# insight-platform/Similari

Hardware: NVIDIA H100
Metric: pair_associations_per_sec (higher is better)
Workload: dtype f32

## Files before the change

### similari_b200/csrc/engine.cu

```cuda
#include <cuda_runtime.h>

#include <algorithm>
#include <chrono>
#include <cmath>
#include <cstdlib>
#include <cstdarg>
#include <cstdio>
#include <cstring>
#include <map>
#include <string>
#include <type_traits>
#include <unordered_map>
#include <utility>
#include <vector>

#include "../../include/similari_b200.h"
#include "sb_engine.cuh"

#include <atomic>

namespace sb {
static std::atomic<unsigned long long> g_launches{0};
void note_launch(int n) { g_launches.fetch_add((unsigned long long)n, std::memory_order_relaxed); }
unsigned long long launch_count() { return g_launches.load(std::memory_order_relaxed); }
// ... 276 lines not shown
    }
    if (copy_stream) cudaStreamDestroy(copy_stream);
    if (side_stream) cudaStreamDestroy(side_stream);
    if (prep_stream) cudaStreamDestroy(prep_stream);
    for (cudaEvent_t e : {ev_user_in, ev_user_out, ev_prep_done, ev_set_free[0], ev_set_free[1], ev_inputs, ev_join_req, ev_cost_done}) if (e) cudaEventDestroy(e);
    for (auto& e : ev_fork) if (e) cudaEventDestroy(e);
    if (ev_join) cudaEventDestroy(ev_join);
    if (own_stream && stream) cudaStreamDestroy(stream);
  }

  template <auto F> static void in_ts(sb200_tracker& t, void* p) { t.ts.*F = static_cast<std::remove_reference_t<decltype(t.ts.*F)>>(p); }
  template <auto F> static void in_wb(sb200_tracker& t, void* p) { t.wb.*F = static_cast<std::remove_reference_t<decltype(t.wb.*F)>>(p); }

  std::vector<Col> store_table() {
    using TS = sb::TrackStore;
    const size_t K = (size_t)P.max_obs, d8 = (size_t)P.d8, H = (size_t)hist_len;
    std::vector<Col> c = {{&b_id, in_ts<&TS::id>, 8}, {&b_epoch, in_ts<&TS::epoch>, 4}, {&b_length, in_ts<&TS::length>, 4},
                          {&b_custom, in_ts<&TS::custom>, 8}, {&b_vt, in_ts<&TS::vt>, 1}, {&b_pred, in_ts<&TS::pred>, 24},
                          {&b_obs, in_ts<&TS::obs>, 24}, {&b_radius, in_ts<&TS::radius>, 4},
                          {&b_kst, in_ts<&TS::kst>, 4 * (size_t)sb::kStateStride}};
    if (P.positional_kind == SB200_POS_IOU) c.push_back({&b_vert, in_ts<&TS::vert>, 64});
    if (H > 1) {
      c.push_back({&b_hpred, in_ts<&TS::hist_pred>, 24 * H, true});
      c.push_back({&b_hobs, in_ts<&TS::hist_obs>, 24 * H, true});
    }
    if (P.is_visual) {
      c.push_back({&b_obs_phys, in_ts<&TS::obs_phys>, K, false, kRowTrack, kBlobAll, kTagObsPhys});
      c.push_back({&b_obs_hasf, in_ts<&TS::obs_hasf>, K});
      c.push_back({&b_obs_q, in_ts<&TS::obs_q>, 4 * K});
      c.push_back({&b_obs_n, in_ts<&TS::obs_n>, 1, false, kRowTrack, kBlobAll, kTagObsN});
      c.push_back({&b_feat_cnt, in_ts<&TS::feat_cnt>, 1});
      c.push_back({&b_fblk, in_ts<&TS::fblk>, 4, false, kRowTrack, kBlobAll, kTagFblk});
      if (fhist_on) c.push_back({&b_hblk, in_ts<&TS::hblk>, 4, false, kRowTrack, kBlobTrackerOnly, kTagHblk});
      c.push_back({&b_feat, in_ts<&TS::feat>, 4 * K * d8, false, kRowBlock});
      c.push_back({&b_feat_bf16, in_ts<&TS::feat_bf16>, 2 * K * d8, false, kRowBlock});
      c.push_back({&b_fnorm2, in_ts<&TS::fnorm2>, 4 * K, false, kRowBlock});
      if (P.d8 <= sb::kFp8MaxD8) {
        c.push_back({&b_feat_fp8, in_ts<&TS::feat_fp8>, K * sb::fp8_pitch(P.d8), false, kRowBlock, kBlobNo});
        c.push_back({&b_fscale, in_ts<&TS::fscale>, 4 * K, false, kRowBlock, kBlobNo});
      }
      c.push_back({&b_blk_owner, in_ts<&TS::blk_owner>, 4, false, kRowBlock, kBlobAll, kTagOwner});
      c.push_back({&b_blk_free, in_ts<&TS::blk_free>, 4, false, kRowFree, kBlobAll, kTagFree});
    }
    return c;
  }

  std::vector<Col> slot_table() {
    using TS = sb::TrackStore;
    return {{&b_ntracks, nullptr, 4, true}, {&b_cur_epoch, nullptr, 4, true}, {&b_scene_ids, nullptr, 8, true},
            {&b_nfree, in_ts<&TS::n_free>, 4, true}, {&b_atop, in_ts<&TS::arena_top>, 4, true}};
  }

  std::vector<Col> wasted_table() {
    using WB = sb::WastedBuf;
    const size_t H = (size_t)hist_len;
    std::vector<Col> c = {{&w_id, in_wb<&WB::id>, 8, false, kRowWasted}, {&w_scene, in_wb<&WB::scene>, 8, false, kRowWasted},
                          {&w_epoch, in_wb<&WB::epoch>, 4, false, kRowWasted}, {&w_length, in_wb<&WB::length>, 4, false, kRowWasted},
                          {&w_pred, in_wb<&WB::pred>, 24, false, kRowWasted}, {&w_obs, in_wb<&WB::obs>, 24, false, kRowWasted}};
    if (H > 1) {
      c.push_back({&w_hpred, in_wb<&WB::hist_pred>, 24 * H, false, kRowWasted});
      c.push_back({&w_hobs, in_wb<&WB::hist_obs>, 24 * H, false, kRowWasted});
    }
    if (fhist_on) c.push_back({&w_hblk, in_wb<&WB::hblk>, 4, false, kRowWasted, kBlobAll, kTagHblk});
    return c;
  }

  std::vector<Col> pool_table() {
    using TS = sb::TrackStore;
// ... 6 lines not shown
  int regrow(DBuf& b, size_t w, size_t groups, size_t rows, size_t old_groups, size_t old_rows, bool zero) {
    const size_t bytes = std::max<size_t>(1, groups * rows * w);
    DBuf nb;
    int rc = nb.ensure(bytes);
    if (rc) return rc;
    if (zero) CU(cudaMemsetAsync(nb.p, 0, bytes, stream));
    if (b.p && old_groups > 0 && old_rows > 0) {
      if (old_groups == 1)
        CU(cudaMemcpyAsync(nb.p, b.p, old_rows * w, cudaMemcpyDeviceToDevice, stream));
      else
        CU(cudaMemcpy2DAsync(nb.p, rows * w, b.p, old_rows * w, old_rows * w, old_groups, cudaMemcpyDeviceToDevice, stream));
      CU(cudaStreamSynchronize(stream));
    }
    b = std::move(nb);
    return 0;
  }

  int grow(const std::vector<Col>& cols, size_t groups, size_t rows, size_t old_groups, size_t old_rows) {
    for (const Col& c : cols) {
      const int rc = regrow(*c.buf, c.w, groups, rows, old_groups, old_rows, c.zero);
      if (rc) return rc;
      if (c.point) c.point(*this, c.buf->p);
    }
    return 0;
  }

  int regen_fp8(int slot, int top) {
    if (!ts.feat_fp8 || top <= 0) return 0;
    const long long r0 = (long long)slot * track_cap * P.max_obs, rows = (long long)top * P.max_obs;
    sb::launch_to_fp8(ts.feat + r0 * P.d8, P.d8, P.d8, P.d8, rows, ts.feat_fp8 + r0 * sb::fp8_pitch(P.d8), ts.fscale + r0, stream);
    return cudaGetLastError() == cudaSuccess ? 0 : fail(SB200_ERR_CUDA, "e4m3 row conversion failed");
  }

  int ensure_store(int need_scenes, int need_tracks) {
    if (need_scenes <= scene_cap && need_tracks <= track_cap) return 0;
    int ns = scene_cap, nt = track_cap;
    if (need_scenes > ns) ns = std::max(need_scenes, std::max(4, ns * 2));
    if (need_tracks > nt) nt = std::max(need_tracks, std::max(64, nt * 2));
    int rc = grow(store_table(), ns, nt, scene_cap, track_cap);
    if (rc) return rc;
    if (ns != scene_cap && (rc = grow(slot_table(), ns, 1, scene_cap, 1))) return rc;
    ts.kst_stride = sb::kStateStride;
    if (hist_len > 1) ts.hist_len = hist_len;
    scene_cap = ns;
    track_cap = nt;
    ts.track_cap = nt;
    return 0;
  }

  int slot_for(uint64_t scene_id, bool create) {
    auto it = slot_of.find(scene_id);
    if (it != slot_of.end()) return it->second;
    if (!create) return -1;
    int s = (int)scene_of_slot.size();
    slot_of[scene_id] = s;
    scene_of_slot.push_back(scene_id);
    epoch.push_back(0);
    n_tracks.push_back(0);
    n_hidden.push_back(0);
    arena_top.push_back(0);
    pending_add.push_back(0);
    return s;
  }

  int ensure_wasted(int64_t need) {
    if (need <= wb.cap) return 0;
    int64_t ncap = std::max<int64_t>(need, std::max<int64_t>(1024, (int64_t)wb.cap * 3));
    int rc = grow(wasted_table(), 1, (size_t)ncap, 1, (size_t)wasted_count);
    if (rc) return rc;
    if (!w_count.p) {
      if ((rc = w_count.ensure(sizeof(int)))) return rc;
      CU(cudaMemsetAsync(w_count.p, 0, sizeof(int), stream));
// ... 440 lines not shown
    if (fhist_on && (rc = ENS(f_histdst, T * 4))) return rc;
    if ((rc = ENS(cb.flags, T)) || (rc = ENS(cb.norm2, T * 4)) || (rc = ENS(f_featdst, T * 4)) ||
        (rc = ENS(f_vis, std::max<size_t>(4, (size_t)vis_total * 4))) || (rc = ENS(f_scene_max, 4 * (size_t)n_scenes)))
      return rc;
  }
  sb::TcArgs tc;
  memset(&tc, 0, sizeof(tc));
  tc.num_sms = num_sms;
  int mstep = 0, cstep = 256;
  const long long visl_alloc = std::max(visl_total, hint_dets * 64);
  if (want_tc || want_dense) {
    tc.use_tc = true;
    tc.dense = want_dense;
    mstep = 256;
    cstep = want_dense ? (256 / K) * K : sb::vis_screen_ucols(P.d8, num_sms, n_scenes, m_of.data(), nb_ub.data(), K);
    tc.cstep = cstep;
    long long tiles_ub = 0, slabs_ub = 0, ws_ub = 0, blk_ub = 0;
    for (int s = 0; s < n_scenes; ++s) {
      const long long ct = ((long long)nb_ub[s] * K + cstep - 1) / cstep;
      tiles_ub += (long long)((m_of[s] + mstep - 1) / mstep) * ct;
      slabs_ub += ct;
      ws_ub += ct * (cstep / K) * ((m_of[s] + 127) / 128 * 128);
      blk_ub += ct * (cstep / K);
    }
    tc.n_tiles = (int)tiles_ub;
    long long tiles_alloc = tiles_ub;
    {
      const long long hs = std::max(opts.max_scenes_hint, n_scenes), hd = std::max(opts.max_dets_per_scene_hint, max_m);
      const long long ht = std::max(hint_tracks, max_nb);
      tiles_alloc = std::max(tiles_alloc, hs * ((hd + mstep - 1) / mstep) * ((ht * K + cstep - 1) / cstep + 1));
      if (f_tiles.bytes > 0 && sizeof(sb::TcTile) * (size_t)tiles_alloc > f_tiles.bytes) tiles_alloc += tiles_alloc / 2;
    }
    const bool alloc8 = !want_dense && P.d8 <= sb::kFp8MaxD8 && ts.feat_fp8 != nullptr;
    if (alloc8 && ((rc = ENS(cb.fp8, T * sb::fp8_pitch(P.d8))) || (rc = ENS(cb.scale, T * 4)))) return rc;
    if ((rc = ENS(cb.bf16, T * P.d8 * 2)) || (rc = ENS(f_tiles, sizeof(sb::TcTile) * (size_t)std::max<long long>(1, tiles_alloc))) ||
        (rc = ENS(f_rowmeta, sizeof(sb::VisRowMeta) * (T + 256))))
      return rc;
    tc.rowmeta = f_rowmeta.as<sb::VisRowMeta>();
    tc.max_rows = max_nb * K;
    tc.d_tiles = f_tiles.as<sb::TcTile>();
    tc.d_n_tiles = &f_dyn.as<sb::FrameDyn>()->n_tiles;
    tc.a_rows = total;
    tc.b_rows = (long long)scene_cap * track_cap * K;
    if (!want_dense) {
      if ((rc = ENS(f_colmeta, sizeof(sb::VisColMeta) * (size_t)(std::max(col_total, hint_cols) + 256))) ||
          (rc = ENS(f_colb, 4 * (size_t)(std::max(col_total, hint_cols) + 256))) ||
          (rc = ENS(f_colvalid, (size_t)(std::max(col_total, hint_cols) + 256) / 8 + 16)) ||
          (rc = ENS(f_colgeo, sizeof(sb::VisColGeo) * (size_t)std::max<long long>(1, P.n_constraints > 0 ? std::max(col_total, hint_cols) : 1))))
        return rc;
      tc.colmeta = f_colmeta.as<sb::VisColMeta>();
      tc.colgeo = f_colgeo.as<sb::VisColGeo>();
      tc.colb = f_colb.as<float>();
      tc.colvalid = f_colvalid.as<unsigned int>();
      tc.total_cols = (int)col_total;
      if (alloc8 && P.visual_kind != SB200_VIS_COSINE) {
        if ((rc = ENS(f_colsb, 4 * (size_t)(std::max(col_total, hint_cols) + 256)))) return rc;
        if (want_fp8) tc.colsb = f_colsb.as<float>();
      }
      tc.fp8 = want_fp8;
    } else {
      const long long hs = std::max(opts.max_scenes_hint, n_scenes), ht = hint_tracks;
      const long long hd = std::max(opts.max_dets_per_scene_hint, 0);
      ws_ub = std::max(ws_ub, hs * (ht + 256) * ((hd + 127) / 128 * 128));
      blk_ub = std::max(blk_ub, hs * (ht + 256));
      slabs_ub = std::max(slabs_ub, hs * ((ht * K + cstep - 1) / cstep + 1));
      if ((rc = ENS(f_drowb, 4 * 5 * T)) || (rc = ENS(f_dcolb, 4 * (size_t)std::max<long long>(1, blk_ub))) ||
          (rc = ENS(f_slabk, 4 * 256 * (size_t)std::max<long long>(1, slabs_ub))))
// ... 162 lines not shown
  } rollback{this, &q, true};

  const double ms_setup = since(t_begin);
  if (has_user_stream) {
    if (!ev_user_in) { CU(cudaEventCreateWithFlags(&ev_user_in, cudaEventDisableTiming)); CU(cudaEventCreateWithFlags(&ev_user_out, cudaEventDisableTiming)); }
    CU(cudaEventRecord(ev_user_in, user_stream));
    CU(cudaStreamWaitEvent(stream, ev_user_in, 0));
  }
  if (!device_io && !prefetched && total > 0) {
    const size_t n = (size_t)total;
    CU(cudaMemcpyAsync(sin->boxes.p, boxes, n * 24, cudaMemcpyHostToDevice, stream));
    if (f.in_feat) {
      CU(cudaMemcpyAsync(sin->feat.p, features, n * (size_t)P.feature_dim * feat_bytes(), cudaMemcpyHostToDevice, stream));
      if (f.in_hasf) CU(cudaMemcpyAsync(sin->hasf.p, has_feature, n, cudaMemcpyHostToDevice, stream));
    }
    if (f.in_quality) CU(cudaMemcpyAsync(sin->quality.p, quality, n * 4, cudaMemcpyHostToDevice, stream));
    if (f.in_custom) CU(cudaMemcpyAsync(sin->custom.p, custom_ids, n * 8, cudaMemcpyHostToDevice, stream));
    if (f.in_own) CU(cudaMemcpyAsync(sin->own.p, own_area, n * 4, cudaMemcpyHostToDevice, stream));
  }
  if (!side_stream) {
    int lo = 0, hi = 0;
    CU(cudaDeviceGetStreamPriorityRange(&lo, &hi));
    CU(cudaStreamCreateWithPriority(&side_stream, cudaStreamNonBlocking, hi));
    for (auto& e : ev_fork) CU(cudaEventCreateWithFlags(&e, cudaEventDisableTiming));
    CU(cudaEventCreateWithFlags(&ev_join, cudaEventDisableTiming));
  }
  if (!prep_stream) {
    int lo = 0, hi = 0;
    CU(cudaDeviceGetStreamPriorityRange(&lo, &hi));
    CU(cudaStreamCreateWithPriority(&prep_stream, cudaStreamNonBlocking, lo));
    CU(cudaEventCreateWithFlags(&ev_prep_done, cudaEventDisableTiming));
    CU(cudaEventCreateWithFlags(&ev_inputs, cudaEventDisableTiming));
  }
  const bool prep_ahead = !derive_own && total > 0;
  const bool side_setup = !derive_own && total > 0;
  cudaStream_t s_setup = stream;
  if (side_setup) {
    CU(cudaEventRecord(ev_fork[0], stream));
    CU(cudaStreamWaitEvent(side_stream, ev_fork[0], 0));
    s_setup = side_stream;
  }
  sb::launch_frame_setup(P, ts, f, reinterpret_cast<const sb::SceneReq*>(q.h_req.dp), n_scenes, b_ntracks.as<int>(), mstep,
                         cstep, tc.dense, f_tiles.as<sb::TcTile>(), f_dyn.as<sb::FrameDyn>(), f_counters.as<int>(), (int)n_counters, s_setup);
  tc.max_init_done = 1;
  if (side_setup && Pf.is_visual && tc.use_tc && !tc.dense && tc.n_tiles > 0 && max_m > 0 && max_n > 0 && f.in_feat) {
    sb::launch_vis_colmeta(Pf, ts, f, n_scenes, max_n, tc, side_stream);
    tc.colmeta_done = 1;
  }
  if (side_setup) CU(cudaEventRecord(ev_join, side_stream));
  CU(cudaEventRecord(q.ev[0], stream));
  if (derive_own) {
    sb::launch_own_area(f, n_scenes, max_m, f.in_boxes, f_own.as<float>(), f_ownovf.as<int>(),
                        reinterpret_cast<int2*>(f_ownovf.as<char>() + 16), stream);
    f.in_own = f_own.as<float>();
  }
  if (prep_ahead) {
    if (has_user_stream) CU(cudaStreamWaitEvent(prep_stream, ev_user_in, 0));
    if (!device_io) {
      if (prefetched) CU(cudaStreamWaitEvent(prep_stream, sin->ev, 0));
      else { CU(cudaEventRecord(ev_inputs, stream)); CU(cudaStreamWaitEvent(prep_stream, ev_inputs, 0)); }
    }
    if (set_busy[cset]) CU(cudaStreamWaitEvent(prep_stream, ev_set_free[cset], 0));
    if (cost_done_valid) CU(cudaStreamWaitEvent(prep_stream, ev_cost_done, 0));
    sb::launch_prep(Pf, f, n_scenes, max_m, prep_stream);
    CU(cudaEventRecord(ev_prep_done, prep_stream));
    CU(cudaStreamWaitEvent(stream, ev_prep_done, 0));
// ... 898 lines not shown
  int bad = 0;
  CU(cudaMemcpyAsync(&bad, d_bad, sizeof(int), cudaMemcpyDeviceToHost, t->stream));
  CU(cudaStreamSynchronize(t->stream));
  if (bad) return fail(SB200_ERR_INVALID, "the blob holds %d out-of-range block or observation indices", bad);
  return 0;
}

int set_slots(sb200_tracker* t, const std::vector<sb::XferSlot>& tab, int free0, int free_add, int top_add,
              unsigned long long id_min, bool raise_ids) {
  if (tab.empty()) return 0;
  DBuf d_tab;
  int rc = d_tab.ensure(tab.size() * sizeof(sb::XferSlot));
  if (rc) return rc;
  CU(cudaMemcpyAsync(d_tab.p, tab.data(), tab.size() * sizeof(sb::XferSlot), cudaMemcpyHostToDevice, t->stream));
  const int e = sb::launch_xfer_slots(d_tab.as<sb::XferSlot>(), (int)tab.size(), t->b_ntracks.as<int>(), t->ts.n_free,
                                      t->ts.arena_top, t->ts, free0, free_add, top_add,
                                      raise_ids ? t->b_idc.as<unsigned long long>() : nullptr, id_min, t->stream);
  if (e) return fail(SB200_ERR_CUDA, "slot update launch failed: %s", cudaGetErrorString((cudaError_t)e));
  CU(cudaStreamSynchronize(t->stream));
  return 0;
}

uint64_t read_id_counter(sb200_tracker* t, int* rc) {
  uint64_t v = 0;
  *rc = 0;
  if (!t->b_idc.p) return 0;
  cudaError_t e = cudaMemcpyAsync(&v, t->b_idc.p, 8, cudaMemcpyDeviceToHost, t->stream);
  if (e == cudaSuccess) e = cudaStreamSynchronize(t->stream);
  if (e != cudaSuccess) *rc = fail(SB200_ERR_CUDA, "id counter read failed: %s", cudaGetErrorString(e));
  return v;
}

int save_blob(sb200_tracker* t, uint32_t type, const std::vector<int>& slots, void* dst, size_t cap, size_t* bytes) {
  BlobHeader h;
  memset(&h, 0, sizeof(h));
  h.magic = kBlobMagic; h.version = kBlobVersion; h.type = type;
  h.opts = t->opts;
  h.feature_history = t->fhist_on; h.hist_len = t->hist_len; h.d8 = t->P.d8; h.n_scenes = (int32_t)slots.size();
  h.seen_features = t->seen_features;
  if (type == kBlobTracker) {
    h.adapt_dense = t->adapt_dense;
    h.auto_waste_counter = t->auto_waste_counter; h.auto_waste_periodicity = t->auto_waste_periodicity;
    h.scene_cap = t->scene_cap; h.track_cap = t->track_cap;
  }
  std::vector<BlobScene> table(slots.size());
  std::vector<SlotRows> rows(slots.size());
  for (size_t i = 0; i < slots.size(); ++i) {
    const int s = slots[i];
    const int blk = t->P.is_visual ? t->arena_top[s] : 0;
    table[i] = {t->scene_of_slot[s], t->epoch[s], t->n_tracks[s], type == kBlobTracker ? t->n_hidden[s] : 0, blk};
    rows[i] = {s, t->n_tracks[s], blk, t->P.is_visual ? blk - t->n_tracks[s] : 0};
    h.live_total += rows[i].n; h.blk_total += rows[i].blk; h.free_total += rows[i].fre;
  }
  if (type == kBlobTracker) {
    h.wasted_count = t->wasted_count; h.revealed = t->revealed;
    h.hpool_top = t->fhist_on ? t->hpool_top : 0; h.hpool_free = t->fhist_on ? t->hpool_free : 0;
    h.hpool_cap = t->fhist_on ? t->hpool_cap : 0;
  }
  int rc = 0;
  h.id_counter = read_id_counter(t, &rc);
  if (rc) return rc;
  const uint64_t total = lay_out(h, section_bytes(t, type, h.n_scenes, h.live_total, h.blk_total, h.free_total,
                                                  h.wasted_count, h.hpool_top, h.hpool_free));
  h.total_bytes = total;
  *bytes = (size_t)total;
  if (!dst || cap < total) return fail(SB200_ERR_CAPACITY, "the blob needs %llu bytes", (unsigned long long)total);
// ... 318 lines not shown
```

### similari_b200/csrc/kernels_state.cu

```cuda
#include <cuda_bf16.h>

#include <algorithm>
#include <type_traits>

#include "sb_engine.cuh"

namespace sb {

constexpr int AT = 512;

__device__ __forceinline__ void write_box(float* dst, const Box& b) {
  dst[0] = b.xc; dst[1] = b.yc; dst[2] = b.angle; dst[3] = b.aspect; dst[4] = b.height; dst[5] = b.conf;
}
__device__ __forceinline__ void write_box_row(float* dst, const Box& b) {
  float2* d2 = reinterpret_cast<float2*>(dst);
  d2[0] = make_float2(b.xc, b.yc); d2[1] = make_float2(b.angle, b.aspect); d2[2] = make_float2(b.height, b.conf);
}

__global__ void __launch_bounds__(AT) apply_rank_kernel(Params p, TrackStore ts, Frame f, int n_scenes, int* n_tracks) {
  __shared__ int s_warp[AT / 32];
  __shared__ int s_carry;
  __shared__ int s_newbefore;
  const int sidx = blockIdx.x;
  const SceneDesc sc = f.scenes[sidx];
// ... 226 lines not shown
      if (isnew) {
        const int r = s_newbefore + rank, hn0 = ts.hpool[0];
        hb = r < hn0 ? ts.hfree[hn0 - 1 - r] : ts.hpool[1] + (r - hn0);
        ts.hblk[idx] = hb;
      } else {
        hb = ts.hblk[idx];
      }
      const size_t hrow = (size_t)hb * ts.fhist_len + (o_len - 1u) % (unsigned int)ts.fhist_len;
      ts.hpresent[hrow] = flags & 1;
      f.hist_dst[g] = (flags & 1) ? (int)hrow : -1;
    }
    if (ts.hist_len > 1) {
      const size_t hslot = (idx * ts.hist_len + (size_t)((o_len - 1u) % (unsigned int)ts.hist_len)) * 6;
      write_box_row(ts.hist_pred + hslot, pred);
      if (isnew) {
        const float* rb2 = f.in_boxes + (size_t)g * 6;
        write_box_row(ts.hist_obs + hslot, Box{rb2[0], rb2[1], rb2[2], rb2[3], rb2[4], rb2[5]});
      } else write_box_row(ts.hist_obs + hslot, cb);
    }
    if (f.o_ids) f.o_ids[g] = o_id;
    if (f.o_epochs) f.o_epochs[g] = sc.epoch;
    if (f.o_lengths) f.o_lengths[g] = o_len;
    if (f.o_vt) f.o_vt[g] = p.is_visual ? (o_vt < 0 ? (unsigned char)1 : (unsigned char)o_vt) : (unsigned char)1;
    if (f.o_pred) write_box(f.o_pred + (size_t)g * 6, pred);
    if (f.o_obs) write_box(f.o_obs + (size_t)g * 6, isnew ? Box{f.in_boxes[(size_t)g * 6], f.in_boxes[(size_t)g * 6 + 1], f.in_boxes[(size_t)g * 6 + 2], f.in_boxes[(size_t)g * 6 + 3], f.in_boxes[(size_t)g * 6 + 4], f.in_boxes[(size_t)g * 6 + 5]} : cb);
  }
}

template <class T>
__global__ void feat_store_kernel(Params p, TrackStore ts, Frame f) {
  int w = (blockIdx.x * blockDim.x + threadIdx.x) >> 5;
  int lane = threadIdx.x & 31;
  if (w >= f.total) return;
  w += f.det0;
  const int dst = f.feat_dst[w];
  const int hdst = f.hist_dst ? f.hist_dst[w] : -1;
  if (dst < 0 && hdst < 0) return;
  const T* src = static_cast<const T*>(f.in_feat) + (size_t)w * p.feature_dim;
  float* d = ts.feat + (size_t)max(dst, 0) * p.d8;
  __nv_bfloat16* db = reinterpret_cast<__nv_bfloat16*>(ts.feat_bf16) + (size_t)max(dst, 0) * p.d8;
  float* hd = hdst >= 0 ? ts.hrows + (size_t)hdst * p.d8 : nullptr;
  if constexpr (!std::is_same<T, float>::value) {
    if (p.feature_dim == p.d8 && (reinterpret_cast<uintptr_t>(f.in_feat) & 15) == 0) {
      const uint4* s8 = reinterpret_cast<const uint4*>(src);
      float4* d4 = reinterpret_cast<float4*>(d);
      float4* h4 = reinterpret_cast<float4*>(hd);
      uint4* b8 = reinterpret_cast<uint4*>(db);
      const int n8 = p.d8 >> 3;
      for (int i0 = 0; i0 < n8; i0 += 128) {
        uint4 r[4];
#pragma unroll
        for (int u = 0; u < 4; ++u) {
          const int i = i0 + u * 32 + lane;
          if (i < n8) r[u] = __ldcs(s8 + i);
        }
#pragma unroll
        for (int u = 0; u < 4; ++u) {
          const int i = i0 + u * 32 + lane;
          if (i < n8) {
            float x[8];
            feat_widen8(r[u], src, x);
            const float4 lo = make_float4(x[0], x[1], x[2], x[3]), hi = make_float4(x[4], x[5], x[6], x[7]);
            if (dst >= 0) {
              d4[2 * i] = lo;
              d4[2 * i + 1] = hi;
              __nv_bfloat162 bb[4];
#pragma unroll
              for (int l = 0; l < 4; ++l) bb[l] = __floats2bfloat162_rn(x[2 * l], x[2 * l + 1]);
              b8[i] = *reinterpret_cast<const uint4*>(bb);
            }
            if (h4) { __stcs(h4 + 2 * i, lo); __stcs(h4 + 2 * i + 1, hi); }
          }
        }
      }
    } else {
      for (int i = lane; i < p.d8; i += 32) {
        float x = i < p.feature_dim ? feat_elem(src, i) : 0.0f;
        if (dst >= 0) {
          d[i] = x;
          db[i] = __float2bfloat16_rn(x);
        }
        if (hd) hd[i] = x;
      }
    }
  } else if (p.feature_dim == p.d8 && (reinterpret_cast<uintptr_t>(f.in_feat) & 15) == 0) {
    const float4* s4 = reinterpret_cast<const float4*>(src);
    float4* d4 = reinterpret_cast<float4*>(d);
    float4* h4 = reinterpret_cast<float4*>(hd);
    uint2* b4 = reinterpret_cast<uint2*>(db);
    const int n4 = p.d8 >> 2;
    for (int i0 = 0; i0 < n4; i0 += 128) {
      float4 v[4];
#pragma unroll
      for (int u = 0; u < 4; ++u) {
        const int i = i0 + u * 32 + lane;
        if (i < n4) v[u] = __ldcs(s4 + i);
      }
#pragma unroll
      for (int u = 0; u < 4; ++u) {
        const int i = i0 + u * 32 + lane;
        if (i < n4) {
          if (dst >= 0) {
            d4[i] = v[u];
            const __nv_bfloat162 lo = __floats2bfloat162_rn(v[u].x, v[u].y), hi = __floats2bfloat162_rn(v[u].z, v[u].w);
            uint2 pk;
            pk.x = *reinterpret_cast<const unsigned int*>(&lo);
            pk.y = *reinterpret_cast<const unsigned int*>(&hi);
            b4[i] = pk;
          }
          if (h4) __stcs(h4 + i, v[u]);
        }
      }
    }
  } else {
    for (int i = lane; i < p.d8; i += 32) {
      float x = i < p.feature_dim ? src[i] : 0.0f;
      if (dst >= 0) {
        d[i] = x;
        db[i] = __float2bfloat16_rn(x);
      }
      if (hd) hd[i] = x;
    }
  }
  if (dst >= 0 && ts.feat_fp8) {
    __syncwarp();
    const float s = fp8_row_from(d, p.d8, p.d8, ts.feat_fp8 + (size_t)dst * fp8_pitch(p.d8));
    if (lane == 0) ts.fscale[dst] = s;
  }
  if (lane == 0 && dst >= 0) ts.fnorm2[dst] = f.c_norm2[w];
}

__global__ void hist_gather_kernel(TrackStore ts, int d8, const int* __restrict__ blk, const unsigned int* __restrict__ lengths,
                                   int n, int hist_cap, float* __restrict__ out_rows, unsigned char* __restrict__ out_present) {
  const long long w = ((long long)blockIdx.x * blockDim.x + threadIdx.x) >> 5;
  const int lane = threadIdx.x & 31;
  if (w >= (long long)n * hist_cap) return;
  const int i = (int)(w / hist_cap), c = (int)(w - (long long)i * hist_cap);
  const unsigned int len = lengths[i], H = (unsigned int)ts.fhist_len;
  const int cnt = (int)min(min(len, H), (unsigned int)hist_cap);
  unsigned char present = 0;
  size_t row = 0;
  if (c < cnt) {
    const unsigned int j = len - (unsigned int)cnt + (unsigned int)c;
    row = (size_t)blk[i] * H + j % H;
    present = ts.hpresent[row];
  }
  if (lane == 0) out_present[w] = present;
  const float4* s4 = reinterpret_cast<const float4*>(ts.hrows + row * d8);
  float4* d4 = reinterpret_cast<float4*>(out_rows + (size_t)w * d8);
  for (int k = lane; k < (d8 >> 2); k += 32) d4[k] = present ? s4[k] : make_float4(0.0f, 0.0f, 0.0f, 0.0f);
}

void launch_hist_gather(const TrackStore& ts, int d8, const int* blk, const unsigned int* lengths, int n, int hist_cap,
                        float* out_rows, unsigned char* out_present, cudaStream_t st) {
  const long long threads = (long long)n * hist_cap * 32;
  if (threads == 0) return;
  hist_gather_kernel<<<(unsigned)((threads + 255) / 256), 256, 0, st>>>(ts, d8, blk, lengths, n, hist_cap, out_rows,
                                                                        out_present);
  note_launch();
}

void launch_apply(const Params& p, const TrackStore& ts, const Frame& f, int n_scenes, int max_m,
// ... 423 lines not shown
```

### similari_b200/csrc/sb_engine.cuh

```cuda
#pragma once
#include <cuda_bf16.h>
#include <cuda_fp16.h>
#include <cuda_fp8.h>
#include <cuda_runtime.h>
#include <stdint.h>

#include "sb_math.cuh"

namespace sb {

constexpr int kMaxConstraints = 8;
constexpr int kNumSms = 132;
constexpr int kMaxObs = 8;
constexpr int kStateStride = 32;
constexpr int kMaxHist = 64;

inline float screen_rel_err(int d) {
  const double e = 0x1p-7 + 0x1p-16 + (double)d * 0x1p-23;
  const float floor_e = 2.1f / 256.0f;
  return e <= (double)floor_e ? floor_e : (float)(e * (1.0 + 0x1p-20));
}

inline float screen_rel_err_fp8(int d) {
  const double u = 0x1p-4;
  const double rnd = 2.0 * u + u * u;
  const double sub = 2.0 * (1.0 + u) * __builtin_sqrt((double)d) * 0x1p-10 / 224.0 + (double)d * 0x1p-20 / (224.0 * 224.0);
  const double acc = (double)((d + 31) / 32) * 34.0 * 0x1p-12 * (1.0 + u) * (1.0 + u) * 1.01;
  return (float)((rnd + sub + acc) * (1.0 + 0x1p-20));
}

__host__ __device__ __forceinline__ bool fp8_norm_ok(float n2) { return n2 >= 0x1p-60f && n2 <= 0x1p60f; }
__host__ __device__ __forceinline__ float fp8_row_scale(float amax) {
  if (!(amax >= 0x1p-100f && amax <= 0x1p100f)) return 1.0f;
  int e = 0;
  const float m = frexpf(amax, &e);
  return ldexpf(1.0f, (m >= 0.875f ? 8 : 9) - e);
}
__host__ __device__ __forceinline__ int fp8_pitch(int d8) { return (d8 + 15) & ~15; }

__device__ __forceinline__ uint2 fp8_pack8(const float* x, float s) {
  unsigned int w[2];
#pragma unroll
  for (int h = 0; h < 2; ++h) {
    const unsigned int lo = __nv_cvt_float2_to_fp8x2(make_float2(x[4 * h] * s, x[4 * h + 1] * s), __NV_SATFINITE, __NV_E4M3);
    const unsigned int hi = __nv_cvt_float2_to_fp8x2(make_float2(x[4 * h + 2] * s, x[4 * h + 3] * s), __NV_SATFINITE, __NV_E4M3);
    w[h] = lo | (hi << 16);
  }
  return make_uint2(w[0], w[1]);
}
__device__ __forceinline__ float fp8_row_store(const float (&x)[2][8], int d8, unsigned char* out) {
  const int lane = threadIdx.x & 31;
  float amax = 0.0f;
#pragma unroll
  for (int h = 0; h < 2; ++h)
#pragma unroll
    for (int l = 0; l < 8; ++l) amax = fmaxf(amax, fabsf(x[h][l]));
#pragma unroll
  for (int o = 16; o > 0; o >>= 1) amax = fmaxf(amax, __shfl_xor_sync(0xffffffffu, amax, o));
  const float s = fp8_row_scale(amax);
#pragma unroll
  for (int h = 0; h < 2; ++h) {
    const int blk = h * 32 + lane;
    if (blk * 8 < d8) *reinterpret_cast<uint2*>(out + blk * 8) = fp8_pack8(x[h], s);
  }
  return s;
}
__device__ __forceinline__ float fp8_row_from(const float* src, int d, int d8, unsigned char* out) {
  const int lane = threadIdx.x & 31;
  float x[2][8];
#pragma unroll
  for (int h = 0; h < 2; ++h)
#pragma unroll
    for (int l = 0; l < 8; ++l) {
      const int c = (h * 32 + lane) * 8 + l;
      x[h][l] = c < d ? src[c] : 0.0f;
    }
  return fp8_row_store(x, d8, out);
}

struct Params {
  int kind, positional_kind, visual_kind;
// ... 135 lines not shown
  int total;
  int det0;
  int scene0;
  int feat_type;
  const int* new_count_all;
  long long pos_fill_off;
  const float* in_boxes;
  const void* in_feat;
  const unsigned char* in_hasf;
  const float* in_quality;
  const long long* in_custom;
  const float* in_own;
  float* c_box;
  float* c_radius;
  float* c_conf;
  double* c_vert;
  unsigned char* c_flags;
  float* c_norm2;
  void* c_bf16;
  unsigned char* c_fp8;
  float* c_scale;
  int* screen_cnt;
  unsigned int* scene_max;
  int* winner;
  unsigned char* c_vt;
  float* pos;
  bool pos_dense_all;
  long long pos_total;
  float* vis;
  SceneDesc* scenes;
  int* new_count;
  int* status;
  int* feat_dst;
  int* hist_dst;
  int2* app_rank;
  int4* app_meta;
  int* frame_out;
  const FrameDyn* dyn;
  unsigned long long* id_counter;
  long long id_add;
  PosEntry* pos_list;
  int* pos_cnt;
  VisPair* vis_pairs;
  float* vis_val;
  int* vis_cnt;
  int* scene_mode;
  int* vis_mode;
  unsigned char* decided;
  unsigned char* excl;
  int* pre_winner;
  int* dense_cnt;
  int* refine_next;
  const int* dense_bad;
  unsigned long long* o_ids;
  unsigned int* o_epochs;
  unsigned int* o_lengths;
  unsigned char* o_vt;
  float* o_pred;
  float* o_obs;
};

struct TcTile { int scene, m0, c0, pad; };
struct VisColMeta {
  float colb;
  float colc;
  int outcol;
// ... 63 lines not shown
int launch_vis_dense(const Params& p, const TrackStore& ts, const Frame& f, int n_scenes, int max_m, const TcArgs& tc,
                     cudaStream_t st);
int launch_vis_cost_a(const Params& p, const TrackStore& ts, const Frame& f, int n_scenes, int max_m, int max_n,
                      const TcArgs& tc, cudaStream_t st);
int launch_vis_cost_b(const Params& p, const TrackStore& ts, const Frame& f, int n_scenes, int max_m, int max_n,
                      const TcArgs& tc, cudaStream_t st);
void launch_pos_fill(const Params& p, const Frame& f, int n_scenes, int max_m, int max_n, cudaStream_t st);
void launch_pos_scan(const Params& p, const TrackStore& ts, const Frame& f, int n_scenes, int max_m, int max_n,
                     cudaStream_t st);
void launch_pos_scan_lazy(const Params& p, const TrackStore& ts, const Frame& f, int n_scenes, int max_m, int max_n,
                          int pass, cudaStream_t st);
int launch_vote_masks(const Params& p, const TrackStore& ts, const Frame& f, int n_scenes, int max_m, int max_n,
                      cudaStream_t st);
void launch_vis_colmeta(const Params& p, const TrackStore& ts, const Frame& f, int n_scenes, int max_n, const TcArgs& tc,
                        cudaStream_t st);
int vis_screen_ucols(int d8, int num_sms, int n_scenes, const int* m, const int* nb, int K);
int launch_vis_cost_tc(const Params& p, const TrackStore& ts, const Frame& f, int n_scenes, int max_n, const TcArgs& tc,
                       int phase, cudaStream_t st);
void launch_vis_densify(const Params& p, const Frame& f, int n_scenes, cudaStream_t st);
void launch_to_bf16(const float* src, int src_pitch, int d, int d8, long long rows, void* dst, cudaStream_t st);
void launch_to_fp8(const float* src, int src_pitch, int d, int d8, long long rows, unsigned char* dst, float* scale,
                   cudaStream_t st);
constexpr int kFp8MaxD8 = 512;
void launch_scene_max(const Params& p, const Frame& f, int n_scenes, bool init_only, cudaStream_t st);
void launch_scene_mode(const Params& p, const Frame& f, int n_scenes, bool tc_used, cudaStream_t st);
void launch_vis_mode(const Params& p, const Frame& f, int n_scenes, bool tc_used, cudaStream_t st);
size_t voting_smem_need(int max_m, int max_n, int viscap = 0);
constexpr size_t kVotingSmemLimit = 220 * 1024;
int launch_voting(const Params& p, const TrackStore& ts, const Frame& f, int n_scenes, int max_m, int max_n,
                  cudaStream_t st);
void launch_apply(const Params& p, const TrackStore& ts, const Frame& f, int n_scenes, int max_m,
                  unsigned long long id_base, int* d_n_tracks, cudaStream_t st);
bool launch_feat_store(const Params& p, const TrackStore& ts, const Frame& f, cudaStream_t st);
struct WastedBuf {
  int cap;
  int* count;
  unsigned long long* id;
  unsigned long long* scene;
  unsigned int* epoch;
  unsigned int* length;
  float* pred;
  float* obs;
  float* hist_pred;
  float* hist_obs;
  int* hblk;
};
void launch_waste(const Params& p, const TrackStore& ts, int n_slots, const unsigned int* d_cur_epoch,
                  const unsigned long long* d_scene_ids, int* d_n_tracks, const WastedBuf& wb, int max_n,
                  cudaStream_t st);
void launch_frame_sweep(const Params& p, const TrackStore& ts, const Frame& f, int n_scenes, int* d_n_tracks,
                        const WastedBuf& wb, cudaStream_t st);
void launch_hist_gather(const TrackStore& ts, int d8, const int* blk, const unsigned int* lengths, int n, int hist_cap,
                        float* out_rows, unsigned char* out_present, cudaStream_t st);

constexpr int kXferChunk = 32 * 1024;
struct XferSeg { const char* src; char* dst; unsigned long long bytes; };
int launch_xfer_copy(const XferSeg* d_segs, const long long* d_cpre, int n_seg, long long chunks, int num_sms,
                     cudaStream_t st);
int launch_xfer_hist(const TrackStore& ts, int d8, const int* d_slots, const int* d_pre, int n, int total, int dir,
                     float* rows, unsigned char* pres, int base, int num_sms, cudaStream_t st);
struct XferSlot { int slot, n_tracks, n_free, arena_top, push, push_off; };
struct XferCheck { const void* p; const unsigned char* aux; long long n; int lo, hi, kind; };
int launch_xfer_check(const XferCheck* d_ck, int n, int K, int* bad, cudaStream_t st);
int launch_xfer_slots(const XferSlot* d_tab, int n, int* d_n_tracks, int* d_n_free, int* d_arena_top,
                      const TrackStore& ts, int free0, int free_add, int top_add, unsigned long long* id_counter,
                      unsigned long long id_min, cudaStream_t st);
// ... 27 lines not shown
```

Baseline: 58.58 billion.

## Defer BF16 feature mirror writes when FP8 path is active, regenerate lazily

When the FP8 tensor-core path is used, the feature store kernel skips writing the BF16 copy of each stored feature row. Instead it logs the destination rows so a regeneration kernel can rebuild the BF16 mirror before a BF16 consumer, a store regrow or a blob save needs it. The FP8 quantisation is also computed from registers already holding the input, instead of reading the FP32 row back from global memory. This cuts global write and read traffic per frame, at the cost of extra bookkeeping, a log buffer, and a risk of stale BF16 data if any consumer is missed.

```diff
diff --git a/similari_b200/csrc/engine.cu b/similari_b200/csrc/engine.cu
--- a/similari_b200/csrc/engine.cu
+++ b/similari_b200/csrc/engine.cu
@@ -332,8 +332,8 @@
       c.push_back({&b_feat_cnt, in_ts<&TS::feat_cnt>, 1});
       c.push_back({&b_fblk, in_ts<&TS::fblk>, 4, false, kRowTrack, kBlobAll, kTagFblk});
       if (fhist_on) c.push_back({&b_hblk, in_ts<&TS::hblk>, 4, false, kRowTrack, kBlobTrackerOnly, kTagHblk});
-      c.push_back({&b_feat, in_ts<&TS::feat>, 4 * K * d8, false, kRowBlock});
-      c.push_back({&b_feat_bf16, in_ts<&TS::feat_bf16>, 2 * K * d8, false, kRowBlock});
+      c.push_back({&b_feat, in_ts<&TS::feat>, 4 * K * d8, true, kRowBlock});
+      c.push_back({&b_feat_bf16, in_ts<&TS::feat_bf16>, 2 * K * d8, true, kRowBlock});
       c.push_back({&b_fnorm2, in_ts<&TS::fnorm2>, 4 * K, false, kRowBlock});
       if (P.d8 <= sb::kFp8MaxD8) {
         c.push_back({&b_feat_fp8, in_ts<&TS::feat_fp8>, K * sb::fp8_pitch(P.d8), false, kRowBlock, kBlobNo});
@@ -406,12 +406,27 @@
     return cudaGetLastError() == cudaSuccess ? 0 : fail(SB200_ERR_CUDA, "e4m3 row conversion failed");
   }
 
+  static constexpr long long kBf16LogCap = 1 << 18;
+  DBuf b_bf16log;
+  long long bf16_log_n = 0;
+  bool bf16_stale_all = false;
+  int regen_bf16() {
+    if (bf16_stale_all) sb::launch_bf16_regen(ts, P.d8, P.max_obs, nullptr, 0, scene_cap, stream);
+    else if (bf16_log_n > 0) sb::launch_bf16_regen(ts, P.d8, P.max_obs, b_bf16log.as<int>(), bf16_log_n, 0, stream);
+    else return 0;
+    bf16_log_n = 0;
+    bf16_stale_all = false;
+    return cudaGetLastError() == cudaSuccess ? 0 : fail(SB200_ERR_CUDA, "BF16 row conversion failed");
+  }
+
   int ensure_store(int need_scenes, int need_tracks) {
     if (need_scenes <= scene_cap && need_tracks <= track_cap) return 0;
     int ns = scene_cap, nt = track_cap;
     if (need_scenes > ns) ns = std::max(need_scenes, std::max(4, ns * 2));
     if (need_tracks > nt) nt = std::max(need_tracks, std::max(64, nt * 2));
-    int rc = grow(store_table(), ns, nt, scene_cap, track_cap);
+    int rc = regen_bf16();
+    if (rc) return rc;
+    rc = grow(store_table(), ns, nt, scene_cap, track_cap);
     if (rc) return rc;
     if (ns != scene_cap && (rc = grow(slot_table(), ns, 1, scene_cap, 1))) return rc;
     ts.kst_stride = sb::kStateStride;
@@ -918,7 +933,8 @@
       if (f_tiles.bytes > 0 && sizeof(sb::TcTile) * (size_t)tiles_alloc > f_tiles.bytes) tiles_alloc += tiles_alloc / 2;
     }
     const bool alloc8 = !want_dense && P.d8 <= sb::kFp8MaxD8 && ts.feat_fp8 != nullptr;
-    if (alloc8 && ((rc = ENS(cb.fp8, T * sb::fp8_pitch(P.d8))) || (rc = ENS(cb.scale, T * 4)))) return rc;
+    if (alloc8 && ((rc = ENS(cb.fp8, T * sb::fp8_pitch(P.d8))) || (rc = ENS(cb.scale, T * 4)) || (rc = ENS(b_bf16log, kBf16LogCap * 4))))
+      return rc;
     if ((rc = ENS(cb.bf16, T * P.d8 * 2)) || (rc = ENS(f_tiles, sizeof(sb::TcTile) * (size_t)std::max<long long>(1, tiles_alloc))) ||
         (rc = ENS(f_rowmeta, sizeof(sb::VisRowMeta) * (T + 256))))
       return rc;
@@ -1147,6 +1163,17 @@
     CU(cudaEventCreateWithFlags(&ev_prep_done, cudaEventDisableTiming));
     CU(cudaEventCreateWithFlags(&ev_inputs, cudaEventDisableTiming));
   }
+  if (q.fp8 && f.in_feat) {
+    f.skip_bf16 = true;
+    if (!bf16_stale_all && bf16_log_n + total <= kBf16LogCap) {
+      f.bf16_log = b_bf16log.as<int>() + bf16_log_n;
+      bf16_log_n += total;
+    } else {
+      bf16_stale_all = true;
+    }
+  } else if (tc.use_tc && !tc.fp8) {
+    if ((rc = regen_bf16())) return rc;
+  }
   const bool prep_ahead = !derive_own && total > 0;
   const bool side_setup = !derive_own && total > 0;
   cudaStream_t s_setup = stream;
@@ -2111,6 +2138,7 @@
 }
 
 int save_blob(sb200_tracker* t, uint32_t type, const std::vector<int>& slots, void* dst, size_t cap, size_t* bytes) {
+  if (int rc = t->regen_bf16()) return rc;
   BlobHeader h;
   memset(&h, 0, sizeof(h));
   h.magic = kBlobMagic; h.version = kBlobVersion; h.type = type;
diff --git a/similari_b200/csrc/kernels_state.cu b/similari_b200/csrc/kernels_state.cu
--- a/similari_b200/csrc/kernels_state.cu
+++ b/similari_b200/csrc/kernels_state.cu
@@ -282,6 +282,7 @@
   int w = (blockIdx.x * blockDim.x + threadIdx.x) >> 5;
   int lane = threadIdx.x & 31;
   if (w >= f.total) return;
+  if (lane == 0 && f.bf16_log) f.bf16_log[w] = f.feat_dst[f.det0 + w];
   w += f.det0;
   const int dst = f.feat_dst[w];
   const int hdst = f.hist_dst ? f.hist_dst[w] : -1;
@@ -289,7 +290,9 @@
   const T* src = static_cast<const T*>(f.in_feat) + (size_t)w * p.feature_dim;
   float* d = ts.feat + (size_t)max(dst, 0) * p.d8;
   __nv_bfloat16* db = reinterpret_cast<__nv_bfloat16*>(ts.feat_bf16) + (size_t)max(dst, 0) * p.d8;
+  const bool wb = dst >= 0 && !f.skip_bf16;
   float* hd = hdst >= 0 ? ts.hrows + (size_t)hdst * p.d8 : nullptr;
+  unsigned char* d8p = dst >= 0 && ts.feat_fp8 ? ts.feat_fp8 + (size_t)dst * fp8_pitch(p.d8) : nullptr;
   if constexpr (!std::is_same<T, float>::value) {
     if (p.feature_dim == p.d8 && (reinterpret_cast<uintptr_t>(f.in_feat) & 15) == 0) {
       const uint4* s8 = reinterpret_cast<const uint4*>(src);
@@ -297,8 +300,8 @@
       float4* h4 = reinterpret_cast<float4*>(hd);
       uint4* b8 = reinterpret_cast<uint4*>(db);
       const int n8 = p.d8 >> 3;
+      uint4 r[4];
       for (int i0 = 0; i0 < n8; i0 += 128) {
-        uint4 r[4];
 #pragma unroll
         for (int u = 0; u < 4; ++u) {
           const int i = i0 + u * 32 + lane;
@@ -314,6 +317,8 @@
             if (dst >= 0) {
               d4[2 * i] = lo;
               d4[2 * i + 1] = hi;
+            }
+            if (wb) {
               __nv_bfloat162 bb[4];
 #pragma unroll
               for (int l = 0; l < 4; ++l) bb[l] = __floats2bfloat162_rn(x[2 * l], x[2 * l + 1]);
@@ -323,14 +328,29 @@
           }
         }
       }
+      if (d8p) {
+        float x[2][8];
+#pragma unroll
+        for (int h = 0; h < 2; ++h) {
+          if (h * 32 + lane < n8) feat_widen8(r[h], src, x[h]);
+          else
+#pragma unroll
+            for (int l = 0; l < 8; ++l) x[h][l] = 0.0f;
+        }
+        const float s = fp8_row_store(x, p.d8, d8p);
+        if (lane == 0) ts.fscale[dst] = s;
+      }
     } else {
       for (int i = lane; i < p.d8; i += 32) {
         float x = i < p.feature_dim ? feat_elem(src, i) : 0.0f;
-        if (dst >= 0) {
-          d[i] = x;
-          db[i] = __float2bfloat16_rn(x);
-        }
+        if (dst >= 0) d[i] = x;
+        if (wb) db[i] = __float2bfloat16_rn(x);
         if (hd) hd[i] = x;
+      }
+      if (d8p) {
+        __syncwarp();
+        const float s = fp8_row_from(d, p.d8, p.d8, d8p);
+        if (lane == 0) ts.fscale[dst] = s;
       }
     }
   } else if (p.feature_dim == p.d8 && (reinterpret_cast<uintptr_t>(f.in_feat) & 15) == 0) {
@@ -339,8 +359,8 @@
     float4* h4 = reinterpret_cast<float4*>(hd);
     uint2* b4 = reinterpret_cast<uint2*>(db);
     const int n4 = p.d8 >> 2;
+    float4 v[4];
     for (int i0 = 0; i0 < n4; i0 += 128) {
-      float4 v[4];
 #pragma unroll
       for (int u = 0; u < 4; ++u) {
         const int i = i0 + u * 32 + lane;
@@ -350,8 +370,8 @@
       for (int u = 0; u < 4; ++u) {
         const int i = i0 + u * 32 + lane;
         if (i < n4) {
-          if (dst >= 0) {
-            d4[i] = v[u];
+          if (dst >= 0) d4[i] = v[u];
+          if (wb) {
             const __nv_bfloat162 lo = __floats2bfloat162_rn(v[u].x, v[u].y), hi = __floats2bfloat162_rn(v[u].z, v[u].w);
             uint2 pk;
             pk.x = *reinterpret_cast<const unsigned int*>(&lo);
@@ -362,22 +382,68 @@
         }
       }
     }
+    if (d8p) {
+      float amax = 0.0f;
+#pragma unroll
+      for (int u = 0; u < 4; ++u)
+        if (u * 32 + lane < n4)
+          amax = fmaxf(amax, fmaxf(fmaxf(fabsf(v[u].x), fabsf(v[u].y)), fmaxf(fabsf(v[u].z), fabsf(v[u].w))));
+#pragma unroll
+      for (int o = 16; o > 0; o >>= 1) amax = fmaxf(amax, __shfl_xor_sync(0xffffffffu, amax, o));
+      const float s = fp8_row_scale(amax);
+      unsigned int* o4 = reinterpret_cast<unsigned int*>(d8p);
+#pragma unroll
+      for (int u = 0; u < 4; ++u) {
+        const int i = u * 32 + lane;
+        if (i < n4) o4[i] = fp8_pack4(v[u].x, v[u].y, v[u].z, v[u].w, s);
+      }
+      if (lane == 0) ts.fscale[dst] = s;
+    }
   } else {
     for (int i = lane; i < p.d8; i += 32) {
       float x = i < p.feature_dim ? src[i] : 0.0f;
-      if (dst >= 0) {
-        d[i] = x;
-        db[i] = __float2bfloat16_rn(x);
-      }
+      if (dst >= 0) d[i] = x;
+      if (wb) db[i] = __float2bfloat16_rn(x);
       if (hd) hd[i] = x;
     }
-  }
-  if (dst >= 0 && ts.feat_fp8) {
-    __syncwarp();
-    const float s = fp8_row_from(d, p.d8, p.d8, ts.feat_fp8 + (size_t)dst * fp8_pitch(p.d8));
-    if (lane == 0) ts.fscale[dst] = s;
+    if (d8p) {
+      __syncwarp();
+      const float s = fp8_row_from(d, p.d8, p.d8, d8p);
+      if (lane == 0) ts.fscale[dst] = s;
+    }
   }
   if (lane == 0 && dst >= 0) ts.fnorm2[dst] = f.c_norm2[w];
+}
+
+__global__ void bf16_regen_kernel(TrackStore ts, int d8, int K, const int* __restrict__ rows, long long n, int n_slots) {
+  const int lane = threadIdx.x & 31, wpb = blockDim.x >> 5;
+  auto convert = [&](long long r) {
+    const float4* s4 = reinterpret_cast<const float4*>(ts.feat + (size_t)r * d8);
+    uint2* b4 = reinterpret_cast<uint2*>(reinterpret_cast<__nv_bfloat16*>(ts.feat_bf16) + (size_t)r * d8);
+    for (int k = lane; k < (d8 >> 2); k += 32) {
+      const float4 v = s4[k];
+      const __nv_bfloat162 lo = __floats2bfloat162_rn(v.x, v.y), hi = __floats2bfloat162_rn(v.z, v.w);
+      b4[k] = make_uint2(*reinterpret_cast<const unsigned int*>(&lo), *reinterpret_cast<const unsigned int*>(&hi));
+    }
+  };
+  const long long w0 = (long long)blockIdx.x * wpb + (threadIdx.x >> 5), ws = (long long)gridDim.x * wpb;
+  if (rows) {
+    for (long long i = w0; i < n; i += ws)
+      if (rows[i] >= 0) convert(rows[i]);
+    return;
+  }
+  for (int s = blockIdx.y; s < n_slots; s += gridDim.y) {
+    const long long r0 = (long long)s * ts.track_cap * K, nr = (long long)ts.arena_top[s] * K;
+    for (long long i = w0; i < nr; i += ws) convert(r0 + i);
+  }
+}
+
+void launch_bf16_regen(const TrackStore& ts, int d8, int K, const int* rows, long long n, int n_slots, cudaStream_t st) {
+  if (rows ? n <= 0 : n_slots <= 0) return;
+  const long long warps = rows ? n : (long long)ts.track_cap * K;
+  const dim3 grid((unsigned)std::min<long long>((warps + 7) / 8, 2048), rows ? 1u : (unsigned)std::min(n_slots, 65535));
+  bf16_regen_kernel<<<grid, 256, 0, st>>>(ts, d8, K, rows, n, n_slots);
+  note_launch();
 }
 
 __global__ void hist_gather_kernel(TrackStore ts, int d8, const int* __restrict__ blk, const unsigned int* __restrict__ lengths,
diff --git a/similari_b200/csrc/sb_engine.cuh b/similari_b200/csrc/sb_engine.cuh
--- a/similari_b200/csrc/sb_engine.cuh
+++ b/similari_b200/csrc/sb_engine.cuh
@@ -38,15 +38,13 @@
 }
 __host__ __device__ __forceinline__ int fp8_pitch(int d8) { return (d8 + 15) & ~15; }
 
+__device__ __forceinline__ unsigned int fp8_pack4(float a, float b, float c, float d, float s) {
+  const unsigned int lo = __nv_cvt_float2_to_fp8x2(make_float2(a * s, b * s), __NV_SATFINITE, __NV_E4M3);
+  const unsigned int hi = __nv_cvt_float2_to_fp8x2(make_float2(c * s, d * s), __NV_SATFINITE, __NV_E4M3);
+  return lo | (hi << 16);
+}
 __device__ __forceinline__ uint2 fp8_pack8(const float* x, float s) {
-  unsigned int w[2];
-#pragma unroll
-  for (int h = 0; h < 2; ++h) {
-    const unsigned int lo = __nv_cvt_float2_to_fp8x2(make_float2(x[4 * h] * s, x[4 * h + 1] * s), __NV_SATFINITE, __NV_E4M3);
-    const unsigned int hi = __nv_cvt_float2_to_fp8x2(make_float2(x[4 * h + 2] * s, x[4 * h + 3] * s), __NV_SATFINITE, __NV_E4M3);
-    w[h] = lo | (hi << 16);
-  }
-  return make_uint2(w[0], w[1]);
+  return make_uint2(fp8_pack4(x[0], x[1], x[2], x[3], s), fp8_pack4(x[4], x[5], x[6], x[7], s));
 }
 __device__ __forceinline__ float fp8_row_store(const float (&x)[2][8], int d8, unsigned char* out) {
   const int lane = threadIdx.x & 31;
@@ -248,6 +246,8 @@
   int* new_count;
   int* status;
   int* feat_dst;
+  bool skip_bf16;
+  int* bf16_log;
   int* hist_dst;
   int2* app_rank;
   int4* app_meta;
@@ -377,6 +377,7 @@
 void launch_apply(const Params& p, const TrackStore& ts, const Frame& f, int n_scenes, int max_m,
                   unsigned long long id_base, int* d_n_tracks, cudaStream_t st);
 bool launch_feat_store(const Params& p, const TrackStore& ts, const Frame& f, cudaStream_t st);
+void launch_bf16_regen(const TrackStore& ts, int d8, int K, const int* rows, long long n, int n_slots, cudaStream_t st);
 struct WastedBuf {
   int cap;
   int* count;
```

New measurement: 60.63 billion (median of 6 runs). +3.5%, better.
